# marionmari/pyGPs

Hardware: AMD Instinct MI355X
Metric: GP fits/sec (nlZ+grad, RBF, N=8192 d=16) (higher is better)
Workload: dtype f64; 1 GPU; GPR+RBF, N=8192 d=16 fp64 synthetic (SURVEY 8d recipe, seed 0), infExact nlZ + dnlZ (BASELINE configs[1]); x,y resident in HBM, hyp changes every step; outputs nlZ, dnlZ(4), alpha(N) to host per step; fits_per_rank=313, fit_streams_per_gpu=2, sched=1

## Files before the change

### pygps_amd/_lib.py

```python
import ctypes as C
import os
import threading

import numpy as np

_HERE = os.path.dirname(os.path.abspath(__file__))
LIB_PATH = os.environ.get("PYGPS_AMD_LIB") or os.path.join(_HERE, "libpygps_amd.so")

COV_RBF, COV_RBFARD, COV_MATERN, COV_RBFUNIT, COV_RQ, COV_PIECEPOLY = 0, 1, 2, 3, 4, 5
COV_RQARD, COV_GABOR, COV_PERIODIC, COV_NOISE, COV_CONST, COV_SM = 6, 7, 8, 9, 10, 11
COV_PRE = 12
COV_LINEAR, COV_POLY, COV_LINARD = 13, 14, 15
COV_COMPOSITE = 100
PROG_LEAF, PROG_SUM, PROG_PRODUCT, PROG_SCALE = 1, 2, 3, 4
PROG_MAX_ARD_DIM = 64
PROG_MAX = 8
MODE_TRAIN, MODE_CROSS, MODE_SELF_TEST = 0, 1, 2
LIK_ERF, LIK_GAUSS, LIK_LAPLACE = 0, 1, 2
ERR_LAPLACE_WNEG = -90
ERR_PROP_NONFINITE = -91
ERR_XU_UNSUPPORTED = -92
PROP_NONE, PROP_T, PROP_SPREAD = 0, 1, 2
PROP_MAX_LABELS = 256
PROP_SORT_LDS = 2048
# ... 78 lines not shown
    "pgp_profile_read": (C.c_int, [_vp, C.c_int, C.POINTER(_i64), _dp, _dp, _dp]),
    "pgp_profile_reset": (C.c_int, [_vp]),
    "pgp_set_option": (C.c_int, [_vp, C.c_char_p, C.c_int]),
    "pgp_comm_unique_id": (C.c_int, [C.c_char_p, C.c_char_p]),
    "pgp_comm_init_rccl": (C.c_int, [_vp, C.c_int, C.c_int, C.c_char_p, C.c_char_p, C.POINTER(_vp)]),
    "pgp_comm_init_host": (C.c_int, [_vp, C.c_int, C.c_int, _vp, _vp, _vp, C.POINTER(_vp)]),
    "pgp_comm_free": (None, [_vp]),
    "pgp_comm_world": (C.c_int, [_vp]),
    "pgp_comm_rank": (C.c_int, [_vp]),
    "pgp_comm_bcast_host": (C.c_int, [_vp, _dp, _i64, C.c_int]),
    "pgp_comm_allreduce_host": (C.c_int, [_vp, _dp, _i64, C.c_int]),
    "pgp_comm_allgather_host": (C.c_int, [_vp, _dp, _i64, _dp]),
    "pgp_sharded_exact_fit": (C.c_int, [_vp, _vp, C.c_int, _dp, C.c_int, C.c_int, C.c_int, C.c_double, _dp, _dp, C.c_int,
                                        C.c_int, _dp, _dp, _dp, _dp, _dp, C.POINTER(_vp)]),
    "pgp_sharded_predict": (C.c_int, [_vp, _vp, _vp, _dp, _i64, _dp, _dp, _dp]),
    "pgp_sfactor_free": (None, [_vp, _vp]),
    "pgp_sfactor_bytes": (_i64, [_vp]),
}

TEST_SIGNATURES = {
    "pgp_test_gemm": (C.c_int, [_vp, C.c_int, C.c_int, C.c_int, C.c_int, C.c_int, C.c_int, C.c_int, C.c_double,
                                C.c_double, _dp, _i64, _dp, _i64, _dp, _i64, C.c_int, C.c_int, C.c_int, C.c_int,
                                _dp]),
    "pgp_test_gemm_shrink": (C.c_int, [_vp, _dp, _i64, C.c_int, C.c_int, C.c_int, C.c_int, C.c_int, C.c_int, _dp, _i64,
                                       _i64]),
    "pgp_test_gemm_zskip": (C.c_int, [_vp] + [C.c_int] * 5 + [C.c_double, C.c_double, _dp, _i64, _dp, _i64, _dp, _dp, _i64,
                                      C.c_int, C.c_int, C.c_int]),
    "pgp_test_gemm_pair": (C.c_int, [_vp, C.c_double, C.c_double, _dp, _i64, _dp, _i64, _dp, _dp, _i64, C.c_int, C.c_int, C.c_int,
                                     C.c_int]),
    "pgp_test_gemm_skip_wait": (C.c_int, [_vp, C.c_int, _dp, _dp, _dp, C.c_int, C.c_int, C.c_int, C.c_int, C.c_int,
                                          C.POINTER(C.c_int)]),
    "pgp_test_probit_hazard": (C.c_int, [_vp, _dp, _dp, C.c_int]),
    "pgp_test_laplace_lik": (C.c_int, [_vp, C.c_int, C.c_double, _dp, _dp, C.c_int, _dp]),
    "pgp_test_laplace_ep_lik": (C.c_int, [_vp, _dp, _dp, _dp, _dp, C.c_int, _dp]),
    "pgp_test_valu_peak": (C.c_int, [_vp, C.c_int, C.c_int, _dp]),
    "pgp_test_mfma_peak": (C.c_int, [_vp, C.c_int, _dp]),
    "pgp_test_mfma_cycles": (C.c_int, [_vp, C.c_int, C.c_int, C.c_int, _dp]),
    "pgp_test_leaf_ticks": (C.c_int, [_vp, _dp]),
    "pgp_test_assemble": (C.c_int, [_vp, C.c_int, C.c_int, _i64, _i64, C.c_int, _dp]),
    "pgp_test_gemm_trace": (C.c_int, [_vp, C.c_int, C.c_int, C.c_int, C.c_int, C.c_int, C.POINTER(C.c_longlong), _i64, C.POINTER(_i64)]),
    "pgp_test_read_gemm_trace": (C.c_int, [_vp, C.POINTER(C.c_longlong), _i64, C.POINTER(_i64)]),
    "pgp_test_store_roof": (C.c_int, [_vp, _i64, C.c_int, C.c_int, _dp]),
    "pgp_test_cumask_gemm": (C.c_int, [_vp, C.c_int, C.c_int, C.c_int, C.c_int, C.c_int, _dp]),
    "pgp_test_wave_costs": (C.c_int, [_vp, _dp]),
    "pgp_test_stream_concurrency": (C.c_int, [_vp, C.c_int, _dp]),
    "pgp_test_slot_probe": (C.c_int, [_vp, C.c_int, C.c_int, C.c_int, C.c_int, C.c_int, C.c_int, _dp]),
# ... 204 lines not shown
```

### pygps_amd/csrc/capi.hip

```cpp
#include <algorithm>
#include <atomic>
#include <cmath>
#include <cstdio>
#include <cstdlib>
#include <cstring>
#include <map>
#include <string>
#include <mutex>
#include <vector>

#include "ctx.h"

static thread_local char g_err[512] = "";
void pgp_set_last_hip_error(hipError_t e, const char* what, const char* file, int line) {
    snprintf(g_err, sizeof(g_err), "HIP error %d (%s) in %s at %s:%d", (int)e, hipGetErrorString(e), what, file, line);
    (void)hipGetLastError();
}

static void ctx_register(pgp_ctx* c);
static void ctx_unregister(pgp_ctx* c);

void prof_collect(pgp_ctx* c) {
    if (c->recs.empty()) return;
    (void)hipStreamSynchronize(c->st);
// ... 132 lines not shown
    (void)hipStreamDestroy(c->st);
    if (c->st2) (void)hipStreamDestroy(c->st2);
    delete c;
}

int pgp_device_info(pgp_ctx* c, int* n_cu, int* sclk_mhz, double* hbm_gib, char* name, int name_len) {
    if (!c) return -1;
    if (n_cu) *n_cu = c->prop.multiProcessorCount;
    if (sclk_mhz) *sclk_mhz = c->prop.clockRate / 1000;
    if (hbm_gib) *hbm_gib = (double)c->prop.totalGlobalMem / (1024.0 * 1024.0 * 1024.0);
    if (name && name_len > 0) { strncpy(name, c->prop.name, name_len - 1); name[name_len - 1] = 0; }
    return PGP_OK;
}

int pgp_set_option(pgp_ctx* c, const char* name, int value) {
    if (!c || !name) return -1;
    if (!strcmp(name, "nb_outer")) { if (value < 0) return -3; c->nb_outer = value; return PGP_OK; }
    if (!strcmp(name, "joint_refine")) { c->joint_refine = value != 0; return PGP_OK; }
    if (!strcmp(name, "small_tile_below")) { c->small_tile_below = value; return PGP_OK; }
    if (!strcmp(name, "trtri_small_tile_below")) { c->trtri_small_tile_below = value; return PGP_OK; }
    if (!strcmp(name, "xcd_order")) { c->xcd_order = value; return PGP_OK; }
    if (!strcmp(name, "gemm_dbg")) { if (value & ~(64 | 256 | 512)) return -2; c->gemm_dbg = value; return PGP_OK; }
    if (!strcmp(name, "tile_ring")) { if (value < 0 || value > 1) return -2; c->tile_ring = value; return PGP_OK; }
    if (!strcmp(name, "lookahead")) { c->lookahead = value; return PGP_OK; }
    if (!strcmp(name, "leaf_first")) { c->leaf_first = value; return PGP_OK; }
    if (!strcmp(name, "leaf_pivot")) { if (value < 0 || value > 2) return -2; c->leaf_pivot = value; return PGP_OK; }
    if (!strcmp(name, "sched")) { if (value < -1 || value > 2) return -2; c->sched = value < 0 ? PGP_SCHED_DEFAULT : value; c->sched_explicit = value >= 0; return PGP_OK; }
    if (!strcmp(name, "concurrent_streams")) { c->concurrent_streams = value != 0; return PGP_OK; }
    if (!strcmp(name, "tud_tile")) { if (value != 64 && value != 128) return -2; c->tud_tile = value; return PGP_OK; }
    if (!strcmp(name, "tur_tile")) { if (value != 0 && value != 64 && value != 128 && value != 1264) return -2; c->tur_tile = value; return PGP_OK; }
    if (!strcmp(name, "s_pan")) { if (value < -1 || value > 2) return -2; c->s_pan = value; return PGP_OK; }
    if (!strcmp(name, "s_pan_direct")) { c->s_pan_direct = value != 0; return PGP_OK; }
    if (!strcmp(name, "s_pan_out")) { c->s_pan_out = value != 0; return PGP_OK; }
    if (!strcmp(name, "skip_zeros")) { c->skip_zeros = value != 0; return PGP_OK; }
    if (!strcmp(name, "tud_mark")) { c->tud_mark = value != 0; return PGP_OK; }
    if (!strcmp(name, "sched2_wide")) { c->sched2_wide = value != 0; return PGP_OK; }
    if (!strcmp(name, "gram_assembly")) { if (value < 0 || value > 2) return -2; c->gram_assembly = value; return PGP_OK; }
    if (!strcmp(name, "yield")) { c->yield = value; return PGP_OK; }
    if (!strcmp(name, "ep_fused")) { c->ep_fused = value; return PGP_OK; }
    if (!strcmp(name, "ep_tol_exp")) { if (value < 1 || value > 16) return -3; c->ep_tol_exp = value; return PGP_OK; }
    if (!strcmp(name, "ep_max_sweep")) { if (value < 2 || value > 1000) return -3; c->ep_max_sweep = value; return PGP_OK; }
    if (!strcmp(name, "laplace_tol_exp")) { if (value < 1 || value > 16) return -3; c->laplace_tol_exp = value; return PGP_OK; }
    if (!strcmp(name, "ep_r_direct")) { c->ep_r_direct = value; return PGP_OK; }
    if (!strcmp(name, "ep_alpha_direct")) { c->ep_alpha_direct = value; return PGP_OK; }
    if (!strcmp(name, "ep_sym")) { c->ep_sym = value; return PGP_OK; }
    if (!strcmp(name, "ep_wait_kernel")) { c->ep_wait_kernel = value; return PGP_OK; }
// ... 395 lines not shown
    for (long k = 0; k < c->d; ++k) bound += cs.scale[k] * cs.scale[k] * c->xdev2[k];
    return bound <= 64.0;
}

static int gemm_prepare(pgp_ctx* c, GemmArgs& g) {
    if (g.batch < 1) g.batch = 1;
    g.dbg |= c->gemm_dbg;
    bool xcd = false;
    if (c->xcd_order && !g.order && g.tile != 64 && g.tile != 1264 && g.batch == 1 && g.K <= c->xcd_max_k) {
        const long mt = g.M / 128, nt = g.N / 128;
        const long tiles = g.tri == 2 ? mt * (mt + 1) / 2 : (g.tri == 1 ? mt * nt - nt * (nt - 1) / 2 : mt * nt);
        xcd = tiles >= c->xcd_min_tiles;
    }
    if (g.tri == 1 && !g.order && !xcd) {
        const int T = g.tile == 64 ? 64 : 128;
        CHK(tri_tile_list(c, g.M / T, g.N / T, g.tri_off / T, &g.order, &g.norder));
    }
    if (xcd) CHK(tile_order(c, g.M / 128, g.N / 128, g.tri, g.tri ? g.tri_off / 128 : 0, &g.order, &g.norder));
    if (c->yield && c->yield_flags) {
        g.yield_flags = c->yield_flags;
        if (g.yield_role != 2) g.yield_role = gemm_f64_uses_dma(g) ? 1 : 0;
    } else g.yield_role = 0;
    g.ring = c->tile_ring && gemm_f64_uses_dma(g) ? 1 : 0;
    if (c->gemm_trace && gemm_f64_uses_dma128(g) && g.batch == 1) {
        const long mt = g.M / 128, nt = g.N / 128;
        const long nb = g.order ? g.norder : (g.tri == 2 ? mt * (mt + 1) / 2 : mt * nt);
        if (c->gemm_trace_pos + nb <= c->gemm_trace_cap) { g.trace = c->gemm_trace + 8 * c->gemm_trace_pos; c->gemm_trace_pos += nb; }
    }
    return PGP_OK;
}

int gemm_prof(pgp_ctx* c, int cls, GemmArgs g, hipStream_t st) {
    if (!st) st = c->st;
    CHK(gemm_prepare(c, g));
    ProfScope ps(c, cls, g.flops, 0.0, st, gemm_f64_uses_dma128(g) ? PC_KERNEL_DMA128 : -1);
    return gemm_f64_launch(g, st);
}

int gemm_prof_pair(pgp_ctx* c, int cls_a, GemmArgs a, int cls_b, GemmArgs b, hipStream_t st) {
    if (!st) st = c->st;
    CHK(gemm_prepare(c, a));
    CHK(gemm_prepare(c, b));
    if (c->pair_launch && gemm_f64_pair_ok(a, b)) {
        ProfScope ps(c, cls_a, a.flops + b.flops, 0.0, st, PC_KERNEL_DMA128);
        return gemm_f64_launch_pair(a, b, st);
    }
// ... 635 lines not shown
```

### pygps_amd/csrc/common.h

```cpp
#pragma once
#include <hip/hip_runtime.h>
#include <cstdint>
#include <cstdio>

#define PGP_OK 0
#define PGP_ERR_HIP (-100)
#define PGP_ERR_ARG (-1)

#define HIP_TRY(expr)                                                                       \
    do {                                                                                    \
        hipError_t e__ = (expr);                                                            \
        if (e__ != hipSuccess) {                                                            \
            pgp_set_last_hip_error(e__, #expr, __FILE__, __LINE__);                         \
            return PGP_ERR_HIP;                                                             \
        }                                                                                   \
    } while (0)

void pgp_set_last_hip_error(hipError_t e, const char* what, const char* file, int line);

enum GemmKMode {
    KM_FULL = 0,
    KM_GE_I = 1,
    KM_GE_J = 2,
    KM_LT_I = 3,
    KM_LT_J = 4,
};

struct GemmArgs {
    const double* A; long lda; int a_kc;
    const double* B; long ldb; int b_kc;
    double* C; long ldc;
    int M, N, K;
    double alpha, beta;
    int tri;
    int tri_off;
    int mask_diag;
    int kmode; int koff;
    int batch; long sA, sB, sC;
    int tile;
    const int* order;
    int norder;
    int order_z;
    int dbg;
    int ring;
    double flops;
    const double* A2; long lda2; int a_split;
    double* C2; long ldc2; int c_split;
    const double* Cin; long ldcin; const double* Cin2; long ldcin2;
    int rev_cols;
    int rev_rows;
    int fold_rows;
    int zero_from;
    int zf_upper;
    int batch_dm;
    int batch_dk;
    int batch_dldc; long batch_sC2;
    unsigned* yield_flags; int yield_role;
    int skip_lo, skip_hi;
    unsigned* wait_flag; unsigned wait_target; unsigned* wait_err;
    long long* trace;
};

__device__ __forceinline__ unsigned pgp_cu_key() {
    const unsigned hw = __builtin_amdgcn_s_getreg((4 << 0) | (0 << 6) | (31 << 11));
    const unsigned xcc = __builtin_amdgcn_s_getreg((20 << 0) | (0 << 6) | (3 << 11)) & 15u;
    return (xcc << 8) | ((hw >> 8) & 0xffu);
}
__device__ __forceinline__ void pgp_yield_mark(unsigned* flags, int delta) {
    if (flags && threadIdx.x == 0) {
        if (delta > 0) __hip_atomic_fetch_add(flags + pgp_cu_key(), 1u, __ATOMIC_RELAXED, __HIP_MEMORY_SCOPE_AGENT);
        else __hip_atomic_fetch_sub(flags + pgp_cu_key(), 1u, __ATOMIC_RELAXED, __HIP_MEMORY_SCOPE_AGENT);
    }
}

int gemm_f64_launch(const GemmArgs& g, hipStream_t st);
bool gemm_f64_pair_ok(const GemmArgs& a, const GemmArgs& b);
int gemm_f64_launch_pair(const GemmArgs& a, const GemmArgs& b, hipStream_t st);
bool gemm_f64_uses_dma(const GemmArgs& g);
bool gemm_f64_uses_dma128(const GemmArgs& g);

void func_max_dynamic_lds(const void* fn, size_t bytes);
```

### pygps_amd/csrc/ctx.h

```cpp
#pragma once
#include <algorithm>
#include <atomic>
#include <chrono>
#include <condition_variable>
#include <cstdio>
#include <cstdlib>
#include <map>
#include <mutex>
#include <vector>

#include "../../include/pygps_amd.h"
#include "kernels.h"
#include "sqdist_tile.h"

enum ProfClass { PC_ASSEMBLE = 0, PC_GEMM_TRAIL, PC_GEMM_INNER, PC_LEAF, PC_TRSM, PC_LEAFINV, PC_GEMM_TRTRI,
                 PC_GEMM_LAUUM, PC_HADAMARD, PC_SMALL, PC_GEMM_SOLVE, PC_DIAG, PC_KERNEL_DMA128, PC_COUNT };
static const char* const kProfNames[PC_COUNT] = {
    "cov_tile_kernel(assemble)", "gemm_f64(potrf trailing syrk)", "gemm_f64(potrf inner update)",
    "leaf_potrf_kernel", "trsm_rows_kernel", "leaf_inv_kernel", "gemm_f64(trtri)", "gemm_f64(lauum W^T W)",
    "hadamard_reduce_kernel", "small/O(N) kernels", "gemm_f64(panel solve X E_D)", "diag_in/out staging",
    "kernel gemm_f64_kernel<128,128,false,false,true,*> + gemm_f64_pair_kernel (LDS-DMA 128-tile)"};

struct ProfRec { int cls; hipEvent_t e0, e1; double flops, bytes; int shadow; };

// ... 101 lines not shown
    double *Dk = nullptr, *dpack = nullptr, *Xs = nullptr;
    int xcd_max_k = 512;
    int xcd_min_tiles = 256;
    int xcd_super = 8;
    int solve_outer = 8;
    int keep_inverse = 1;
    int predict_inverse = 1;
    int joint_refine = 1;
    int predict_batch = 65536;
    int s_tile = 0;
    int gram_fast = 2, gram_grid = 32768;
    int asm_grid = 4096, asm_nt = 0;
    size_t Xs_bytes = 0;
    hipEvent_t ev[PGP_NSTAGE + 2];
    double last_ms[PGP_NSTAGE];
    bool prof = false;
    std::vector<ProfRec> recs;
    std::vector<hipEvent_t> ev_pool;
    double pc_ms[PC_COUNT], pc_flops[PC_COUNT], pc_bytes[PC_COUNT];
    int64_t pc_launch[PC_COUNT];
    std::map<std::vector<int>, std::pair<int*, int>> orders;
    int gemm_dbg = 64 | 256 | 512;
    int tile_ring = 1;
    int xcd_order = 0;
    int nb_outer = 0;
    int trtri_small_tile_below = 2049;
    int small_tile_below = 200;
};

#define CHK(x)                      \
    do {                            \
        int rc__ = (x);             \
        if (rc__ != PGP_OK) return rc__; \
    } while (0)

int pgp_ctx_count_on_device(int device);
void pgp_drop_idle_pools(int device);

static inline bool pool_trace_on() { static const bool on = getenv("PGP_POOL_TRACE") != nullptr; return on; }
static inline hipError_t pool_hip_malloc(void** out, size_t bytes, const char* who) {
    if (!pool_trace_on()) return hipMalloc(out, bytes);
    const auto t0 = std::chrono::steady_clock::now();
    const hipError_t e = hipMalloc(out, bytes);
    fprintf(stderr, "[pool] hipMalloc %8.1f MiB  %8.3f ms  (%s)%s\n", bytes / 1048576.0,
            std::chrono::duration<double, std::milli>(std::chrono::steady_clock::now() - t0).count(), who, e == hipSuccess ? "" : " FAILED");
    return e;
// ... 282 lines not shown
```

### pygps_amd/csrc/gemm_f64.hip

```cpp
#include <algorithm>
#include <atomic>

#include "gemm_tile.h"

void func_max_dynamic_lds(const void* fn, size_t bytes) {
    constexpr int MAXF = 64, MAXD = 16;
    static std::atomic<const void*> fns[MAXF];
    static std::atomic<size_t> done[MAXF][MAXD];
    int dev = 0;
    if (hipGetDevice(&dev) != hipSuccess || dev < 0 || dev >= MAXD) { (void)hipFuncSetAttribute(fn, hipFuncAttributeMaxDynamicSharedMemorySize, (int)bytes); return; }
    int slot = -1;
    for (int i = 0; i < MAXF; ++i) {
        const void* cur = fns[i].load(std::memory_order_acquire);
        if (cur == fn) { slot = i; break; }
        if (cur == nullptr) {
            const void* expect = nullptr;
            if (fns[i].compare_exchange_strong(expect, fn, std::memory_order_acq_rel) || expect == fn) { slot = i; break; }
        }
    }
    if (slot < 0) { (void)hipFuncSetAttribute(fn, hipFuncAttributeMaxDynamicSharedMemorySize, (int)bytes); return; }
    if (done[slot][dev].load(std::memory_order_acquire) >= bytes) return;
    (void)hipFuncSetAttribute(fn, hipFuncAttributeMaxDynamicSharedMemorySize, (int)bytes);
    size_t prev = done[slot][dev].load(std::memory_order_relaxed);
    while (prev < bytes && !done[slot][dev].compare_exchange_weak(prev, bytes, std::memory_order_release)) {}
// ... 6 lines not shown

__device__ __forceinline__ bool decode_tile(const GemmArgs& g, int b, int T, int TNc, int& ti, int& tj) {
    if (g.order) {
        ti = g.order[2 * b];
        tj = g.order[2 * b + 1];
        return ti >= 0;
    }
    if (g.tri == 2) {
        int r = (int)((sqrt(8.0 * (double)b + 1.0) - 1.0) * 0.5);
        while ((long)(r + 1) * (r + 2) / 2 <= b) ++r;
        while ((long)r * (r + 1) / 2 > b) --r;
        ti = r;
        tj = b - r * (r + 1) / 2;
        return true;
    }
    const int mt = g.M / T;
    ti = b % mt;
    tj = b / mt;
    if (g.rev_cols) tj = g.N / TNc - 1 - tj;
    if (g.rev_rows) ti = mt - 1 - ti;
    return true;
}

template <int TM, int TN, bool AKC, bool BKC, bool DMA = false, bool YIELD = false, bool RING = false>
__global__ __launch_bounds__(256, 2) void gemm_f64_kernel(GemmArgs g) {
    extern __shared__ __attribute__((aligned(16))) double smem[];
    if (g.trace) {
        long long* tr0 = g.trace + 8L * (blockIdx.x + (long)gridDim.x * blockIdx.z);
        tr0[0] = (long long)wall_clock64();
        tr0[6] = (long long)__builtin_readcyclecounter();
    }
    int ti, tj;
    if (!decode_tile(g, (int)blockIdx.x, TM, TN, ti, tj)) return;
    long bz = blockIdx.z;
    if (g.order_z) { bz = ti >> 16; ti &= 0xffff; }
    if (g.wait_flag) {
        if (threadIdx.x == 0) {
            for (unsigned it = 0; (int)(__hip_atomic_load(g.wait_flag, __ATOMIC_ACQUIRE, __HIP_MEMORY_SCOPE_AGENT) - g.wait_target) < 0; ++it) {
                if (it > (1u << 22) || ((it & 1023u) == 1023u && __hip_atomic_load(g.wait_err, __ATOMIC_RELAXED, __HIP_MEMORY_SCOPE_AGENT))) {
                    __hip_atomic_store(g.wait_err, 1u, __ATOMIC_RELAXED, __HIP_MEMORY_SCOPE_AGENT);
                    break;
                }
                __builtin_amdgcn_s_sleep(8);
            }
        }
        __syncthreads();
    }
    if (!YIELD && g.yield_role == 2) {
        pgp_yield_mark(g.yield_flags, +1);
        gemm_tile_ns::gemm_tile<TM, TN, AKC, BKC, DMA, false, RING>(g, ti, tj, bz, smem, (int)(blockIdx.x + gridDim.x * blockIdx.z));
        __syncthreads();
        pgp_yield_mark(g.yield_flags, -1);
        return;
    }
    gemm_tile_ns::gemm_tile<TM, TN, AKC, BKC, DMA, YIELD, RING>(g, ti, tj, bz, smem, (int)(blockIdx.x + gridDim.x * blockIdx.z));
}

template <bool YIELD, bool RING = false>
__global__ __launch_bounds__(256, 2) void gemm_f64_pair_kernel(GemmArgs a, GemmArgs b, int na) {
    extern __shared__ __attribute__((aligned(16))) double smem[];
    auto run = [&](const GemmArgs& g, int bid) {
        if (g.trace) {
            long long* tr0 = g.trace + 8L * bid;
            tr0[0] = (long long)wall_clock64();
            tr0[6] = (long long)__builtin_readcyclecounter();
        }
        int ti, tj;
        if (!decode_tile(g, bid, 128, 128, ti, tj)) return;
        gemm_tile_ns::gemm_tile<128, 128, false, false, true, YIELD, RING>(g, ti, tj, 0, smem, bid);
    };
    if ((int)blockIdx.x < na) run(a, (int)blockIdx.x);
    else run(b, (int)blockIdx.x - na);
}

template <bool YIELD, bool RING = false>
__global__ __launch_bounds__(256, 2) void gemm_f64_fold_kernel(GemmArgs g) {
    extern __shared__ __attribute__((aligned(16))) double smem[];
    const int mt = g.M / 128, half = (mt + 1) / 2;
    const int r = (int)blockIdx.x % half, tj = (int)blockIdx.x / half;
    const int hi = mt - 1 - r;
    const long bz = blockIdx.z;
    gemm_tile_ns::gemm_tile<128, 128, false, false, true, YIELD, RING>(g, hi, tj, bz, smem, 0);
    if (hi != r) {
        __syncthreads();
        gemm_tile_ns::gemm_tile<128, 128, false, false, true, YIELD, RING>(g, r, tj, bz, smem, 0);
    }
}

constexpr size_t DMA_SPARE = 16;

template <int T, bool AKC, bool BKC, bool DMA = false, bool YIELD = false, bool RING = false>
int launch_t(const GemmArgs& g, hipStream_t st) {
    constexpr int SK = BK + 2;
    constexpr int ASZ = AKC ? T * SK : BK * (T + 16);
    constexpr int BSZ = BKC ? T * SK : BK * (T + 16);
    const size_t shm = 2 * (ASZ + BSZ) * sizeof(double) + (DMA ? DMA_SPARE : 0);
    const int mt = g.M / T, nt = g.N / T;
    unsigned nblk = (g.tri == 2) ? (unsigned)((long)mt * (mt + 1) / 2) : (unsigned)(mt * nt);
    if (g.order) nblk = (unsigned)g.norder;
    dim3 grid(nblk, 1, (g.batch > 0 && !g.order_z) ? g.batch : 1);
    func_max_dynamic_lds((const void*)gemm_f64_kernel<T, T, AKC, BKC, DMA, YIELD, RING>, shm);
    hipLaunchKernelGGL((gemm_f64_kernel<T, T, AKC, BKC, DMA, YIELD, RING>), grid, dim3(256), shm, st, g);
    return hipGetLastError() == hipSuccess ? PGP_OK : PGP_ERR_HIP;
}

static bool dma_ok(const GemmArgs& g);
static bool dma1264_ok(const GemmArgs& g) {
    return g.tile == 1264 && dma_ok(g) && !g.tri && !g.order && g.batch <= 1 && !g.order_z && (g.N % 64) == 0 && (g.M % 128) == 0 && g.kmode == KM_FULL;
}
template <bool YIELD, bool RING>
int launch_1264(const GemmArgs& g, hipStream_t st) {
    constexpr int SA_ = 128 + 16;
    const size_t shm = 2 * (BK * SA_ + (BK / 2) * SA_) * sizeof(double) + DMA_SPARE;
    dim3 grid((unsigned)((g.M / 128) * (g.N / 64)), 1, 1);
    func_max_dynamic_lds((const void*)gemm_f64_kernel<128, 64, false, false, true, YIELD, RING>, shm);
    hipLaunchKernelGGL((gemm_f64_kernel<128, 64, false, false, true, YIELD, RING>), grid, dim3(256), shm, st, g);
    return hipGetLastError() == hipSuccess ? PGP_OK : PGP_ERR_HIP;
}

static bool dma_ok(const GemmArgs& g) {
    return g.tile != 64 && (g.dbg & 64) && !g.a_kc && !g.b_kc && (g.K % 16) == 0 && (g.koff % 16) == 0 && (g.batch_dk % 16) == 0;
}

template <int T>
int launch_l(const GemmArgs& g, hipStream_t st) {
    if (!g.a_kc && !g.b_kc) return launch_t<T, false, false>(g, st);
    if (!g.a_kc && g.b_kc) return launch_t<T, false, true>(g, st);
    if (g.a_kc && !g.b_kc) return launch_t<T, true, false>(g, st);
    return launch_t<T, true, true>(g, st);
}

}

bool gemm_f64_uses_dma128(const GemmArgs& g) { return dma_ok(g) && !dma1264_ok(g); }
bool gemm_f64_uses_dma(const GemmArgs& g) { return dma_ok(g); }

static unsigned launch_blocks(const GemmArgs& g) {
    const int mt = g.M / 128, nt = g.N / 128;
    if (g.order) return (unsigned)g.norder;
    return (g.tri == 2) ? (unsigned)((long)mt * (mt + 1) / 2) : (unsigned)(mt * nt);
}
bool gemm_f64_pair_ok(const GemmArgs& a, const GemmArgs& b) {
    auto plain = [](const GemmArgs& g) {
        return g.M > 0 && g.N > 0 && g.tile != 64 && dma_ok(g) && g.batch <= 1 && !g.order_z && !g.wait_flag && g.yield_role != 2;
    };
    return plain(a) && plain(b) && (a.yield_role == 1 && a.yield_flags) == (b.yield_role == 1 && b.yield_flags) && !a.ring == !b.ring;
}
int gemm_f64_launch_pair(const GemmArgs& a, const GemmArgs& b, hipStream_t st) {
    if (!gemm_f64_pair_ok(a, b)) return -2;
    constexpr int SA_ = 128 + 16;
    const size_t shm = 2 * (2 * BK * SA_) * sizeof(double) + DMA_SPARE;
    const unsigned na = launch_blocks(a), nb = launch_blocks(b);
    const bool yield = a.yield_role == 1 && a.yield_flags;
    auto go = [&](auto kern) {
        func_max_dynamic_lds((const void*)kern, shm);
        hipLaunchKernelGGL(kern, dim3(na + nb), dim3(256), shm, st, a, b, (int)na);
    };
// ... 37 lines not shown
```

### pygps_amd/csrc/gemm_tile.h

```cpp
#pragma once
#include "common.h"

typedef double double4_t __attribute__((ext_vector_type(4)));
typedef double double2_t __attribute__((ext_vector_type(2)));

namespace gemm_tile_ns {

constexpr int BK = 16;

template <int LDS_OFF>
__device__ __forceinline__ void lds_dma_1k_s(unsigned voff, const double* sbase, unsigned lds_wave_base) {
    asm volatile("s_add_u32 m0, %2, %3\n\ts_nop 0\n\tglobal_load_lds_dwordx4 %0, %1"
                 :: "v"(voff), "s"(sbase), "s"(lds_wave_base), "n"(LDS_OFF) : "memory", "scc");
}
__device__ __forceinline__ const double* uniform_ptr(const double* p) {
    const unsigned long a = (unsigned long)p;
    const unsigned lo = __builtin_amdgcn_readfirstlane((unsigned)a), hi = __builtin_amdgcn_readfirstlane((unsigned)(a >> 32));
    return (const double*)(((unsigned long)hi << 32) | lo);
}
template <int V> struct IC { static constexpr int value = V; };

template <int N>
__device__ __forceinline__ void ring_wait() { asm volatile("s_waitcnt vmcnt(%0)" :: "n"(N) : "memory"); }
template <int N>
// ... 1 lines not shown
    asm volatile("s_waitcnt vmcnt(%0) lgkmcnt(0)" :: "n"(N) : "memory");
    __builtin_amdgcn_s_barrier();
    asm volatile("" ::: "memory");
}
__device__ __forceinline__ void ring_load_f64(double& d, const double* p) {
    asm volatile("global_load_dwordx2 %0, %1, off" : "=v"(d) : "v"(p) : "memory");
}
__device__ __forceinline__ void ring_landed(double& d) { asm volatile("" : "+v"(d)); }
__device__ __forceinline__ void ring_landed(unsigned& d) { asm volatile("" : "+v"(d)); }

__device__ __forceinline__ double swap_adjacent(double v) {
    const int lo = __builtin_amdgcn_update_dpp(0, __double2loint(v), 0xB1, 0xF, 0xF, false);
    const int hi = __builtin_amdgcn_update_dpp(0, __double2hiint(v), 0xB1, 0xF, 0xF, false);
    return __hiloint2double(hi, lo);
}

__device__ __noinline__ void gemm_yield_wait(const unsigned* yf) {
    for (int i = 0; i < 400; ++i) {
        __builtin_amdgcn_s_sleep(32);
        if (__hip_atomic_load(yf, __ATOMIC_RELAXED, __HIP_MEMORY_SCOPE_AGENT) == 0u) break;
    }
}

template <int TM, int TN, bool AKC, bool BKC, bool DMA = false, bool YIELD = false, bool RING = false>
__device__ __forceinline__ void gemm_tile(const GemmArgs& g, int ti, int tj, long bz, double* __restrict__ smem, int wg = 0) {
    static_assert(!RING || DMA, "the staging ring is an LDS-DMA loop");
    static_assert(!DMA || (!AKC && !BKC && TM == 128 && (TN == 128 || TN == 64)), "LDS-DMA staging: M-contiguous operands, 128 x 128 or 128 x 64 tiles");
    constexpr bool BH = DMA && TN == 64;
    constexpr int SA = TM + 16, SB = BH ? TM + 16 : TN + 16, SK = BK + 2;
    constexpr int ASZ = AKC ? TM * SK : BK * SA;
    constexpr int BSZ = BKC ? TN * SK : (BH ? (BK / 2) * SB : BK * SB);
    constexpr int STAGE = ASZ + BSZ;
    constexpr int FM = TM / 32, FN = TN / 32;
    constexpr int AV = TM * BK / 2 / 256;
    constexpr int BV = TN * BK / 2 / 256;

    const int i0 = ti * TM, j0 = tj * TN;
    if (g.batch_dm && i0 >= g.M - (int)bz * g.batch_dm) return;
    const int zero_from = g.zero_from > 0 ? g.zero_from - (int)bz * g.batch_dm : 0;
    if (i0 < g.skip_hi && j0 < g.skip_hi && i0 >= g.skip_lo && j0 >= g.skip_lo) return;
    bool diag = false;
    if (g.tri) {
        if (i0 + g.tri_off < j0) return;
        diag = g.mask_diag && (i0 + g.tri_off == j0);
    }
    int k0 = 0, k1 = g.K;
    const int koff = g.koff + (int)bz * g.batch_dk;
    if (g.kmode == KM_GE_I) k0 = i0 + koff;
    else if (g.kmode == KM_GE_J) k0 = j0 + koff;
// ... 141 lines not shown
                *(double2_t*)(sa + kr * SA + 2 * mv) = ra[p];
            }
        } else {
#pragma unroll
            for (int p = 0; p < AV; ++p) {
                const int kp = t & 7, m = (t >> 3) + p * 32;
                *(double2_t*)(sa + m * SK + 2 * kp) = ra[p];
            }
        }
        if (!BKC) {
            constexpr int VPR = TN / 2;
            constexpr int RPP = 256 / VPR;
#pragma unroll
            for (int p = 0; p < BV; ++p) {
                const int nv = t % VPR, kr = t / VPR + p * RPP;
                *(double2_t*)(sb + kr * SB + 2 * nv) = rb[p];
            }
        } else {
#pragma unroll
            for (int p = 0; p < BV; ++p) {
                const int kp = t & 7, n = (t >> 3) + p * 32;
                *(double2_t*)(sb + n * SK + 2 * kp) = rb[p];
            }
        }
    };

    double cr[8];
    const int ring_half = __builtin_amdgcn_readfirstlane(wave >> 1);
    auto ring_cact = [&](int fold_step) __attribute__((always_inline)) { return !BH || ring_half == (fold_step >> 3); };
    auto ring_cload = [&](int chunk) __attribute__((always_inline)) {
        const int in = chunk / (FM / 2), hf = chunk % (FM / 2);
#pragma unroll
        for (int q = 0; q < 2; ++q) {
            const double* cp = Cin + (long)(i0 + wm + (2 * hf + q) * 16 + l15) + (long)(j0 + wn + in * 16 + l4) * ldcin;
#pragma unroll
            for (int r = 0; r < 4; ++r) ring_load_f64(cr[4 * q + r], cp + (long)(4 * r) * ldcin);
        }
    };
    if (k0 < k1) {
        if constexpr (RING) {
            ring_issue(IC<0>{}, IC<0>{});
            ring_issue(IC<0>{}, IC<1>{});
            if (k0 + BK < k1) {
                ring_issue(IC<1>{}, IC<0>{});
                if (lazyc && ring_cact(1)) { ring_cload(0); ring_wait_barrier<2 * P + 8>(); }
                else ring_wait_barrier<2 * P>();
            } else ring_wait_barrier<P>();
        } else {
        if constexpr (DMA) {
            dma_stage(IC<0>{});
            asm volatile("s_waitcnt vmcnt(0)" ::: "memory");
        } else {
            gload(k0);
            sstore(0);
        }
        __syncthreads();
        }
        double fa[2][FM], fb[2][FN];
        auto ldfrag = [&](int b, int ks, int slot) {
            const double* sa = smem + b * STAGE;
            const double* sb = sa + ASZ;
            const int k = ks * 4 + l4;
#pragma unroll
            for (int im = 0; im < FM; ++im) {
                const int m = wm + im * 16 + l15;
                fa[slot][im] = AKC ? sa[m * SK + k] : sa[k * SA + m];
            }
#pragma unroll
            for (int in = 0; in < FN; ++in) {
                const int n = wn + in * 16 + l15;
                if constexpr (BH) fb[slot][in] = sb[(l4 + 4 * (ks >> 1)) * SB + (ks & 1) * 64 + n];
                else fb[slot][in] = BKC ? sb[n * SK + k] : sb[k * SB + n];
            }
        };
        auto mfmas = [&](int slot) {
#pragma unroll
            for (int in = 0; in < FN; ++in)
#pragma unroll
                for (int im = 0; im < FM; ++im)
// ... 130 lines not shown
                    if (!(st & 1)) {
                        if (act) {
#pragma unroll
                        for (int q = 0; q < 2; ++q) {
                            const double* cp = Cin + (long)(i0 + wm + (2 * hf + q) * 16 + l15) + (long)(j0 + wn + in * 16 + l4) * ldcin;
#pragma unroll
                            for (int r = 0; r < 4; ++r) creg[q][r] = cp[(long)(4 * r) * ldcin];
                        }
                        }
                    } else if (act) {
#pragma unroll
                        for (int q = 0; q < 2; ++q)
#pragma unroll
                            for (int r = 0; r < 4; ++r) acc[2 * hf + q][in][r] = fma(ab, creg[q][r], acc[2 * hf + q][in][r]);
                    }
                    if (st & 1) kstep(kt, IC<1>{}, IC<0>{});
                    else if ((st & 3) == 0) kstep(kt, IC<0>{}, IC<1>{});
                    else kstep(kt, IC<0>{}, IC<0>{});
                    kt += BK;
                }
                if (g.trace) smem[2 * STAGE] = __longlong_as_double((long long)wall_clock64());
            }
        }
        while (kt < k1) {
            kstep(kt, IC<0>{}, IC<1>{});
            kt += BK;
            if (kt >= k1) break;
            kstep(kt, IC<1>{}, IC<0>{});
            kt += BK;
            if constexpr (YIELD) {
                if (kt >= k1) break;
                kstep(kt, IC<0>{}, IC<0>{});
                kt += BK;
                if (kt >= k1) break;
                kstep(kt, IC<1>{}, IC<0>{});
                kt += BK;
            }
        }
        }
    }

    long long* const trc = g.trace ? g.trace + 8L * wg : nullptr;
    if (trc) {
        trc[2] = (long long)wall_clock64();
        if constexpr (DMA) trc[1] = lazyc ? __double_as_longlong(smem[2 * STAGE]) : 0ll;
    }
// ... 42 lines not shown
```

### pygps_amd/csrc/testhooks.h

```cpp
#pragma once
#include <stdint.h>

#include "../../include/pygps_amd.h"
#ifdef __cplusplus
extern "C" {
#endif
int pgp_test_gemm(pgp_ctx* ctx, int tile, int a_kc, int b_kc, int tri, int mask_diag, int kmode, int koff,
                  double alpha, double beta, const double* A, int64_t lda, const double* B, int64_t ldb,
                  double* C, int64_t ldc, int M, int N, int K, int iters, double* ms_out);
int pgp_test_gemm_shrink(pgp_ctx* ctx, const double* Y, int64_t ldy, int M, int K, int w, int nb, int dm, int zero_from,
                         double* C, int64_t ldc, int64_t sC);
int pgp_test_gemm_zskip(pgp_ctx* ctx, int tile, int tri, int mask_diag, int zero_from, int zf_upper, double alpha, double beta,
                        const double* A, int64_t lda, const double* B, int64_t ldb, const double* Cin, double* C, int64_t ldc,
                        int M, int N, int K);
int pgp_test_gemm_pair(pgp_ctx* ctx, double alpha, double beta, const double* A, int64_t lda, const double* B, int64_t ldb, double* Ca,
                       double* Cb, int64_t ldc, int M, int N, int Ka, int Kb);
int pgp_test_gemm_skip_wait(pgp_ctx* ctx, int tile, const double* A, const double* B, double* C, int n, int K, int skip_lo,
                            int skip_hi, int wait_ms, int* timed_out);
int pgp_test_probit_hazard(pgp_ctx* ctx, const double* z, double* out, int n);
int pgp_test_laplace_lik(pgp_ctx* ctx, int lik, double log_sn, const double* y, const double* f, int n, double* out);
int pgp_test_laplace_ep_lik(pgp_ctx* ctx, const double* y, const double* mu, const double* s2, const double* sn, int n, double* out);
int pgp_test_valu_peak(pgp_ctx* ctx, int iters, int waves_per_simd, double* out2);
int pgp_test_mfma_peak(pgp_ctx* ctx, int iters, double* tflops_out);
int pgp_test_mfma_cycles(pgp_ctx* ctx, int iters, int nacc, int waves_per_simd, double* out3);
int pgp_test_leaf_ticks(pgp_ctx* ctx, double* ticks_out );
int pgp_test_wave_costs(pgp_ctx* ctx, double* out16);
int pgp_test_slot_probe(pgp_ctx* ctx, int nwg, int lds_kb, int hold_us, int reserve, int probe_lds_kb, int delay_us, double* out4);
int pgp_test_cumask_gemm(pgp_ctx* ctx, int M, int K, int reserve_per_xcd, int stride, int iters, double* out2);
int pgp_test_assemble(pgp_ctx* ctx, int kind, int mode, int64_t n, int64_t d, int iters, double* ms_out);
int pgp_test_gemm_trace(pgp_ctx* ctx, int M, int K, int tri, int warm, int conc, long long* out, int64_t out_words, int64_t* nblk_out);
int pgp_test_read_gemm_trace(pgp_ctx* ctx, long long* out, int64_t words, int64_t* nwg);
int pgp_test_store_roof(pgp_ctx* ctx, int64_t n, int grid, int iters, double* out3);
// ... 17 lines not shown
```

### pygps_amd/csrc/testhooks.hip

```cpp
#include <time.h>
#include <cstdlib>
#include <cmath>
#include <vector>

#include "ctx.h"
#include <chrono>
#include <thread>

#include "testhooks.h"
#include "erf_lik.h"
#include "laplace_lik.h"

typedef double double4_t __attribute__((ext_vector_type(4)));

namespace {
__global__ __launch_bounds__(256) void mfma_peak_kernel(double* out, int iters, double a0, double b0) {
    double4_t acc[8];
#pragma unroll
    for (int i = 0; i < 8; ++i) acc[i] = double4_t{0.0, 0.0, 0.0, 0.0};
    double a = a0 + threadIdx.x * 1e-9, b = b0;
    for (int it = 0; it < iters; ++it) {
#pragma unroll
        for (int i = 0; i < 8; ++i) acc[i] = __builtin_amdgcn_mfma_f64_16x16x4f64(a, b, acc[i], 0, 0, 0);
    }
// ... 345 lines not shown
    (void)hipEventDestroy(e0); (void)hipEventDestroy(e1);
    (void)hipFree(tab); (void)hipFree(out);
    return hipGetLastError() == hipSuccess ? PGP_OK : PGP_ERR_HIP;
}

int pgp_test_gemm(pgp_ctx* ctx, int tile, int a_kc, int b_kc, int tri, int mask_diag, int kmode, int koff,
                  double alpha, double beta, const double* A, int64_t lda, const double* B, int64_t ldb, double* C,
                  int64_t ldc, int M, int N, int K, int iters, double* ms_out) {
    if (!ctx) return -1;
    pgp_ctx* c = ctx;
    const bool poll = getenv("PGP_TEST_GEMM_YIELD") != nullptr;
    if (poll && !c->yield_flags) return -2;
    HIP_TRY(hipSetDevice(c->device));
    const size_t an = (size_t)lda * (a_kc ? M : K), bn = (size_t)ldb * (b_kc ? N : K), cn = (size_t)ldc * N;
    double *Ad, *Bd, *Cd;
    HIP_TRY(hipMalloc((void**)&Ad, an * 8)); HIP_TRY(hipMalloc((void**)&Bd, bn * 8)); HIP_TRY(hipMalloc((void**)&Cd, cn * 8));
    HIP_TRY(hipMemcpy(Ad, A, an * 8, hipMemcpyHostToDevice));
    HIP_TRY(hipMemcpy(Bd, B, bn * 8, hipMemcpyHostToDevice));
    HIP_TRY(hipMemcpy(Cd, C, cn * 8, hipMemcpyHostToDevice));
    GemmArgs g{};
    g.A = Ad; g.lda = lda; g.a_kc = a_kc; g.B = Bd; g.ldb = ldb; g.b_kc = b_kc; g.C = Cd; g.ldc = ldc;
    g.M = M; g.N = N; g.K = K; g.alpha = alpha; g.beta = beta; g.tri = tri; g.tri_off = 0; g.mask_diag = mask_diag;
    g.kmode = kmode; g.koff = koff; g.batch = 1; g.tile = tile; g.dbg = c->gemm_dbg; g.ring = c->tile_ring != 0;
    if (getenv("PGP_TEST_GEMM_FOLD")) g.fold_rows = 1;
    if (poll && gemm_f64_uses_dma(g)) { g.yield_flags = c->yield_flags; g.yield_role = 1; }
    hipStream_t ts = c->st;
    int rc = gemm_f64_launch(g, ts);
    HIP_TRY(hipStreamSynchronize(ts));
    if (rc == PGP_OK) HIP_TRY(hipMemcpy(C, Cd, cn * 8, hipMemcpyDeviceToHost));
    if (rc == PGP_OK && iters > 0 && ms_out) {
        hipEvent_t e0, e1;
        HIP_TRY(hipEventCreate(&e0)); HIP_TRY(hipEventCreate(&e1));
        {
            HIP_TRY(hipEventRecord(e0, ts));
            rc = gemm_f64_launch(g, ts);
            HIP_TRY(hipEventRecord(e1, ts));
            HIP_TRY(hipStreamSynchronize(ts));
            float m1 = 0.f;
            HIP_TRY(hipEventElapsedTime(&m1, e0, e1));
            const int nwarm = (int)std::min(4000.0, std::max(1.0, 80.0 / std::max(1e-3, (double)m1)));
            for (int i = 0; i < nwarm && rc == PGP_OK; ++i) rc = gemm_f64_launch(g, ts);
        }
        HIP_TRY(hipEventRecord(e0, ts));
        for (int i = 0; i < iters; ++i) rc = gemm_f64_launch(g, ts);
        HIP_TRY(hipEventRecord(e1, ts));
        HIP_TRY(hipStreamSynchronize(ts));
        float ms = 0.f;
        HIP_TRY(hipEventElapsedTime(&ms, e0, e1));
        *ms_out = ms / iters;
        (void)hipEventDestroy(e0); (void)hipEventDestroy(e1);
    }
    (void)hipFree(Ad); (void)hipFree(Bd); (void)hipFree(Cd);
    return rc;
}

int pgp_test_gemm_trace(pgp_ctx* c, int M, int K, int tri, int warm, int conc, long long* out, int64_t out_words, int64_t* nblk_out) {
    if (!c || !out || !nblk_out || M % 128 || K % 16) return -1;
    HIP_TRY(hipSetDevice(c->device));
    const long mt = M / 128;
    const long nblk = tri ? mt * (mt + 1) / 2 : mt * mt;
    if (out_words < 8 * nblk) return -2;
    double *A, *Cd, *C2; long long* tr;
    HIP_TRY(hipMalloc((void**)&A, (size_t)M * K * 8)); HIP_TRY(hipMalloc((void**)&Cd, (size_t)M * M * 8));
    HIP_TRY(hipMalloc((void**)&C2, (size_t)M * M * 8)); HIP_TRY(hipMalloc((void**)&tr, (size_t)nblk * 64));
    HIP_TRY(hipMemset(tr, 0, (size_t)nblk * 64));
    std::vector<double> h((size_t)M * K);
    unsigned long long s = 88172645463325252ULL;
    for (auto& v : h) { s ^= s << 13; s ^= s >> 7; s ^= s << 17; v = ((double)(s >> 11) / 9007199254740992.0 - 0.5) * 0.01; }
    HIP_TRY(hipMemcpy(A, h.data(), h.size() * 8, hipMemcpyHostToDevice));
    HIP_TRY(hipMemset(Cd, 0, (size_t)M * M * 8)); HIP_TRY(hipMemset(C2, 0, (size_t)M * M * 8));
    GemmArgs g{};
    g.A = A; g.lda = M; g.B = A; g.ldb = M; g.C = Cd; g.ldc = M; g.M = M; g.N = M; g.K = K; g.alpha = -1.0; g.beta = 1.0;
    g.tri = tri ? 2 : 0; g.mask_diag = tri ? 1 : 0; g.batch = 1; g.tile = 128; g.dbg = c->gemm_dbg; g.ring = c->tile_ring != 0;
    int rc = PGP_OK;
    for (int i = 0; i < warm && rc == PGP_OK; ++i) rc = gemm_f64_launch(g, c->st);
// ... 396 lines not shown
```

Before: 112.2 fits/s.

## Prefetch global tiles two stages ahead in the register-staged 64x64 GEMM

Adds an AHEAD variant of the 64x64 register-staged f64 GEMM tile. It keeps two sets of staging registers so global loads for the tile after next are issued while the current tile's MFMAs run, which hides more global-memory latency. The variant is enabled by default for tile=64 with a non-transposed A and a K-contiguous B, and its launch bounds go from 2 to 4 waves per unit. The extra staging registers combined with the tighter launch bound could cause spills. The change also adds a test hook for timing and tracing the solve-style GEMM.

```diff
diff --git a/pygps_amd/_lib.py b/pygps_amd/_lib.py
--- a/pygps_amd/_lib.py
+++ b/pygps_amd/_lib.py
@@ -124,6 +124,8 @@
     "pgp_test_gemm": (C.c_int, [_vp, C.c_int, C.c_int, C.c_int, C.c_int, C.c_int, C.c_int, C.c_int, C.c_double,
                                 C.c_double, _dp, _i64, _dp, _i64, _dp, _i64, C.c_int, C.c_int, C.c_int, C.c_int,
                                 _dp]),
+    "pgp_test_gemm_solve": (C.c_int, [_vp, C.c_int, C.c_int, C.c_int, C.c_int, _dp, _i64, _dp, _i64, _dp, _i64, _dp, _i64, C.c_int,
+                                      C.c_int, C.c_int, C.c_int, _dp, C.POINTER(C.c_longlong), _i64]),
     "pgp_test_gemm_shrink": (C.c_int, [_vp, _dp, _i64, C.c_int, C.c_int, C.c_int, C.c_int, C.c_int, C.c_int, _dp, _i64,
                                        _i64]),
     "pgp_test_gemm_zskip": (C.c_int, [_vp] + [C.c_int] * 5 + [C.c_double, C.c_double, _dp, _i64, _dp, _i64, _dp, _dp, _i64,
diff --git a/pygps_amd/csrc/capi.hip b/pygps_amd/csrc/capi.hip
--- a/pygps_amd/csrc/capi.hip
+++ b/pygps_amd/csrc/capi.hip
@@ -178,6 +178,7 @@
     if (!strcmp(name, "xcd_order")) { c->xcd_order = value; return PGP_OK; }
     if (!strcmp(name, "gemm_dbg")) { if (value & ~(64 | 256 | 512)) return -2; c->gemm_dbg = value; return PGP_OK; }
     if (!strcmp(name, "tile_ring")) { if (value < 0 || value > 1) return -2; c->tile_ring = value; return PGP_OK; }
+    if (!strcmp(name, "tile_ahead")) { if (value < 0 || value > 1) return -2; c->tile_ahead = value; return PGP_OK; }
     if (!strcmp(name, "lookahead")) { c->lookahead = value; return PGP_OK; }
     if (!strcmp(name, "leaf_first")) { c->leaf_first = value; return PGP_OK; }
     if (!strcmp(name, "leaf_pivot")) { if (value < 0 || value > 2) return -2; c->leaf_pivot = value; return PGP_OK; }
@@ -619,6 +620,7 @@
         if (g.yield_role != 2) g.yield_role = gemm_f64_uses_dma(g) ? 1 : 0;
     } else g.yield_role = 0;
     g.ring = c->tile_ring && gemm_f64_uses_dma(g) ? 1 : 0;
+    g.ahead = c->tile_ahead ? 1 : 0;
     if (c->gemm_trace && gemm_f64_uses_dma128(g) && g.batch == 1) {
         const long mt = g.M / 128, nt = g.N / 128;
         const long nb = g.order ? g.norder : (g.tri == 2 ? mt * (mt + 1) / 2 : mt * nt);
diff --git a/pygps_amd/csrc/common.h b/pygps_amd/csrc/common.h
--- a/pygps_amd/csrc/common.h
+++ b/pygps_amd/csrc/common.h
@@ -43,6 +43,7 @@
     int order_z;
     int dbg;
     int ring;
+    int ahead;
     double flops;
     const double* A2; long lda2; int a_split;
     double* C2; long ldc2; int c_split;
@@ -78,5 +79,6 @@
 int gemm_f64_launch_pair(const GemmArgs& a, const GemmArgs& b, hipStream_t st);
 bool gemm_f64_uses_dma(const GemmArgs& g);
 bool gemm_f64_uses_dma128(const GemmArgs& g);
+bool gemm_f64_uses_ahead(const GemmArgs& g);
 
 void func_max_dynamic_lds(const void* fn, size_t bytes);
diff --git a/pygps_amd/csrc/ctx.h b/pygps_amd/csrc/ctx.h
--- a/pygps_amd/csrc/ctx.h
+++ b/pygps_amd/csrc/ctx.h
@@ -147,6 +147,7 @@
     std::map<std::vector<int>, std::pair<int*, int>> orders;
     int gemm_dbg = 64 | 256 | 512;
     int tile_ring = 1;
+    int tile_ahead = 1;
     int xcd_order = 0;
     int nb_outer = 0;
     int trtri_small_tile_below = 2049;
diff --git a/pygps_amd/csrc/gemm_f64.hip b/pygps_amd/csrc/gemm_f64.hip
--- a/pygps_amd/csrc/gemm_f64.hip
+++ b/pygps_amd/csrc/gemm_f64.hip
@@ -52,8 +52,8 @@
     return true;
 }
 
-template <int TM, int TN, bool AKC, bool BKC, bool DMA = false, bool YIELD = false, bool RING = false>
-__global__ __launch_bounds__(256, 2) void gemm_f64_kernel(GemmArgs g) {
+template <int TM, int TN, bool AKC, bool BKC, bool DMA = false, bool YIELD = false, bool RING = false, bool AHEAD = false>
+__global__ __launch_bounds__(256, AHEAD ? 4 : 2) void gemm_f64_kernel(GemmArgs g) {
     extern __shared__ __attribute__((aligned(16))) double smem[];
     if (g.trace) {
         long long* tr0 = g.trace + 8L * (blockIdx.x + (long)gridDim.x * blockIdx.z);
@@ -78,12 +78,12 @@
     }
     if (!YIELD && g.yield_role == 2) {
         pgp_yield_mark(g.yield_flags, +1);
-        gemm_tile_ns::gemm_tile<TM, TN, AKC, BKC, DMA, false, RING>(g, ti, tj, bz, smem, (int)(blockIdx.x + gridDim.x * blockIdx.z));
+        gemm_tile_ns::gemm_tile<TM, TN, AKC, BKC, DMA, false, RING, AHEAD>(g, ti, tj, bz, smem, (int)(blockIdx.x + gridDim.x * blockIdx.z));
         __syncthreads();
         pgp_yield_mark(g.yield_flags, -1);
         return;
     }
-    gemm_tile_ns::gemm_tile<TM, TN, AKC, BKC, DMA, YIELD, RING>(g, ti, tj, bz, smem, (int)(blockIdx.x + gridDim.x * blockIdx.z));
+    gemm_tile_ns::gemm_tile<TM, TN, AKC, BKC, DMA, YIELD, RING, AHEAD>(g, ti, tj, bz, smem, (int)(blockIdx.x + gridDim.x * blockIdx.z));
 }
 
 template <bool YIELD, bool RING = false>
@@ -119,7 +119,7 @@
 
 constexpr size_t DMA_SPARE = 16;
 
-template <int T, bool AKC, bool BKC, bool DMA = false, bool YIELD = false, bool RING = false>
+template <int T, bool AKC, bool BKC, bool DMA = false, bool YIELD = false, bool RING = false, bool AHEAD = false>
 int launch_t(const GemmArgs& g, hipStream_t st) {
     constexpr int SK = BK + 2;
     constexpr int ASZ = AKC ? T * SK : BK * (T + 16);
@@ -129,8 +129,8 @@
     unsigned nblk = (g.tri == 2) ? (unsigned)((long)mt * (mt + 1) / 2) : (unsigned)(mt * nt);
     if (g.order) nblk = (unsigned)g.norder;
     dim3 grid(nblk, 1, (g.batch > 0 && !g.order_z) ? g.batch : 1);
-    func_max_dynamic_lds((const void*)gemm_f64_kernel<T, T, AKC, BKC, DMA, YIELD, RING>, shm);
-    hipLaunchKernelGGL((gemm_f64_kernel<T, T, AKC, BKC, DMA, YIELD, RING>), grid, dim3(256), shm, st, g);
+    func_max_dynamic_lds((const void*)gemm_f64_kernel<T, T, AKC, BKC, DMA, YIELD, RING, AHEAD>, shm);
+    hipLaunchKernelGGL((gemm_f64_kernel<T, T, AKC, BKC, DMA, YIELD, RING, AHEAD>), grid, dim3(256), shm, st, g);
     return hipGetLastError() == hipSuccess ? PGP_OK : PGP_ERR_HIP;
 }
 
@@ -154,6 +154,7 @@
 
 template <int T>
 int launch_l(const GemmArgs& g, hipStream_t st) {
+    if constexpr (T == 64) { if (gemm_f64_uses_ahead(g)) return launch_t<64, false, true, false, false, false, true>(g, st); }
     if (!g.a_kc && !g.b_kc) return launch_t<T, false, false>(g, st);
     if (!g.a_kc && g.b_kc) return launch_t<T, false, true>(g, st);
     if (g.a_kc && !g.b_kc) return launch_t<T, true, false>(g, st);
@@ -163,6 +164,7 @@
 }
 
 bool gemm_f64_uses_dma128(const GemmArgs& g) { return dma_ok(g) && !dma1264_ok(g); }
+bool gemm_f64_uses_ahead(const GemmArgs& g) { return g.ahead && g.tile == 64 && !g.a_kc && g.b_kc; }
 bool gemm_f64_uses_dma(const GemmArgs& g) { return dma_ok(g); }
 
 static unsigned launch_blocks(const GemmArgs& g) {
diff --git a/pygps_amd/csrc/gemm_tile.h b/pygps_amd/csrc/gemm_tile.h
--- a/pygps_amd/csrc/gemm_tile.h
+++ b/pygps_amd/csrc/gemm_tile.h
@@ -47,9 +47,10 @@
     }
 }
 
-template <int TM, int TN, bool AKC, bool BKC, bool DMA = false, bool YIELD = false, bool RING = false>
+template <int TM, int TN, bool AKC, bool BKC, bool DMA = false, bool YIELD = false, bool RING = false, bool AHEAD = false>
 __device__ __forceinline__ void gemm_tile(const GemmArgs& g, int ti, int tj, long bz, double* __restrict__ smem, int wg = 0) {
     static_assert(!RING || DMA, "the staging ring is an LDS-DMA loop");
+    static_assert(!AHEAD || (!DMA && !YIELD && TM == 64 && TN == 64), "two stages ahead: the register-staged 64 x 64 tile");
     static_assert(!DMA || (!AKC && !BKC && TM == 128 && (TN == 128 || TN == 64)), "LDS-DMA staging: M-contiguous operands, 128 x 128 or 128 x 64 tiles");
     constexpr bool BH = DMA && TN == 64;
     constexpr int SA = TM + 16, SB = BH ? TM + 16 : TN + 16, SK = BK + 2;
@@ -237,6 +238,28 @@
                 const int kp = t & 7, n = (t >> 3) + p * 32;
                 *(double2_t*)(sb + n * SK + 2 * kp) = rb[p];
             }
+        }
+    };
+    double2_t ra2[AHEAD ? AV : 1], rb2[AHEAD ? BV : 1];
+    auto gload_to = [&](double2_t (&a)[AV], double2_t (&b)[BV], bool adv) __attribute__((always_inline)) {
+        const long sa_ = adv ? astep : 0, sb_ = adv ? bstep : 0;
+#pragma unroll
+        for (int p = 0; p < AV; ++p) { pa[p] += sa_; a[p] = *(const double2_t*)pa[p]; }
+#pragma unroll
+        for (int p = 0; p < BV; ++p) { pb[p] += sb_; b[p] = *(const double2_t*)pb[p]; }
+    };
+    auto sstore_from = [&](int buf, const double2_t (&a)[AV], const double2_t (&b)[BV]) __attribute__((always_inline)) {
+        double* sa = smem + buf * STAGE;
+        double* sb = sa + ASZ;
+#pragma unroll
+        for (int p = 0; p < AV; ++p) {
+            if (!AKC) { constexpr int VPR = TM / 2, RPP = 256 / VPR; *(double2_t*)(sa + (t / VPR + p * RPP) * SA + 2 * (t % VPR)) = a[p]; }
+            else *(double2_t*)(sa + ((t >> 3) + p * 32) * SK + 2 * (t & 7)) = a[p];
+        }
+#pragma unroll
+        for (int p = 0; p < BV; ++p) {
+            if (!BKC) { constexpr int VPR = TN / 2, RPP = 256 / VPR; *(double2_t*)(sb + (t / VPR + p * RPP) * SB + 2 * (t % VPR)) = b[p]; }
+            else *(double2_t*)(sb + ((t >> 3) + p * 32) * SK + 2 * (t & 7)) = b[p];
         }
     };
 
@@ -265,11 +288,18 @@
         if constexpr (DMA) {
             dma_stage(IC<0>{});
             asm volatile("s_waitcnt vmcnt(0)" ::: "memory");
+        } else if constexpr (AHEAD) {
+            gload_to(ra, rb, false);
+            if (k0 + BK < k1) { gload_to(ra2, rb2, true); sstore_from(0, ra, rb); }
+            else sstore_from(0, ra, rb);
         } else {
             gload(k0);
             sstore(0);
         }
         __syncthreads();
+        if constexpr (!DMA && TM == 64 && TN == 64) {
+            if (g.trace) g.trace[8L * wg + 1] = (long long)wall_clock64();
+        }
         }
         double fa[2][FM], fb[2][FN];
         auto ldfrag = [&](int b, int ks, int slot) {
@@ -446,6 +476,31 @@
                 if (g.trace) smem[2 * STAGE] = __longlong_as_double((long long)wall_clock64());
             }
         }
+        if constexpr (AHEAD) {
+            auto astage = [&](auto bufc, auto ldc_, double2_t (&na)[AV], double2_t (&nb)[BV], double2_t (&fra)[AV], double2_t (&frb)[BV])
+                              __attribute__((always_inline)) {
+                constexpr int buf = decltype(bufc)::value, LD = decltype(ldc_)::value;
+                const bool more = kt + BK < k1;
+                if constexpr (LD != 0) gload_to(fra, frb, LD == 1 || kt + 2 * BK < k1);
+#pragma unroll
+                for (int ks = 0; ks + 1 < NS; ++ks) {
+                    ldfrag(buf, ks + 1, (ks + 1) & 1);
+                    mfmas(ks & 1);
+                }
+                if (LD != 0 || more) sstore_from(buf ^ 1, na, nb);
+                __syncthreads();
+                if (LD != 0 || more) ldfrag(buf ^ 1, 0, NS & 1);
+                __builtin_amdgcn_sched_barrier(0);
+                mfmas((NS - 1) & 1);
+                kt += BK;
+            };
+            while (kt + 2 * BK < k1) {
+                astage(IC<0>{}, IC<1>{}, ra2, rb2, ra, rb);
+                astage(IC<1>{}, IC<2>{}, ra, rb, ra2, rb2);
+            }
+            astage(IC<0>{}, IC<0>{}, ra2, rb2, ra, rb);
+            if (kt < k1) astage(IC<1>{}, IC<0>{}, ra, rb, ra2, rb2);
+        } else
         while (kt < k1) {
             kstep(kt, IC<0>{}, IC<1>{});
             kt += BK;
diff --git a/pygps_amd/csrc/testhooks.h b/pygps_amd/csrc/testhooks.h
--- a/pygps_amd/csrc/testhooks.h
+++ b/pygps_amd/csrc/testhooks.h
@@ -8,6 +8,9 @@
 int pgp_test_gemm(pgp_ctx* ctx, int tile, int a_kc, int b_kc, int tri, int mask_diag, int kmode, int koff,
                   double alpha, double beta, const double* A, int64_t lda, const double* B, int64_t ldb,
                   double* C, int64_t ldc, int M, int N, int K, int iters, double* ms_out);
+int pgp_test_gemm_solve(pgp_ctx* ctx, int koff, int c_split, int rev_cols, int ahead, const double* A, int64_t lda, const double* B,
+                        int64_t ldb, double* C, int64_t ldc, double* C2, int64_t ldc2, int M, int N, int K, int iters, double* ms_out,
+                        long long* trace_out, int64_t trace_words);
 int pgp_test_gemm_shrink(pgp_ctx* ctx, const double* Y, int64_t ldy, int M, int K, int w, int nb, int dm, int zero_from,
                          double* C, int64_t ldc, int64_t sC);
 int pgp_test_gemm_zskip(pgp_ctx* ctx, int tile, int tri, int mask_diag, int zero_from, int zf_upper, double alpha, double beta,
diff --git a/pygps_amd/csrc/testhooks.hip b/pygps_amd/csrc/testhooks.hip
--- a/pygps_amd/csrc/testhooks.hip
+++ b/pygps_amd/csrc/testhooks.hip
@@ -391,6 +391,7 @@
     g.A = Ad; g.lda = lda; g.a_kc = a_kc; g.B = Bd; g.ldb = ldb; g.b_kc = b_kc; g.C = Cd; g.ldc = ldc;
     g.M = M; g.N = N; g.K = K; g.alpha = alpha; g.beta = beta; g.tri = tri; g.tri_off = 0; g.mask_diag = mask_diag;
     g.kmode = kmode; g.koff = koff; g.batch = 1; g.tile = tile; g.dbg = c->gemm_dbg; g.ring = c->tile_ring != 0;
+    g.ahead = c->tile_ahead != 0;
     if (getenv("PGP_TEST_GEMM_FOLD")) g.fold_rows = 1;
     if (poll && gemm_f64_uses_dma(g)) { g.yield_flags = c->yield_flags; g.yield_role = 1; }
     hipStream_t ts = c->st;
@@ -420,6 +421,65 @@
         (void)hipEventDestroy(e0); (void)hipEventDestroy(e1);
     }
     (void)hipFree(Ad); (void)hipFree(Bd); (void)hipFree(Cd);
+    return rc;
+}
+
+int pgp_test_gemm_solve(pgp_ctx* c, int koff, int c_split, int rev_cols, int ahead, const double* A, int64_t lda, const double* B,
+                        int64_t ldb, double* C, int64_t ldc, double* C2, int64_t ldc2, int M, int N, int K, int iters, double* ms_out,
+                        long long* trace_out, int64_t trace_words) {
+    if (!c || !A || !B || !C || M <= 0 || N <= 0 || K <= 0 || (M % 64) || (N % 64) || (K % 16)) return -1;
+    if (c_split < 0 || c_split >= M || (c_split % 64) || (c_split > 0 && !C2) || lda < M || ldb < K) return -1;
+    const int m1 = c_split > 0 ? c_split : M, m2 = c_split > 0 ? M - c_split : 0;
+    if (ldc < m1 || (m2 > 0 && ldc2 < m2)) return -1;
+    const long nblk = (long)(M / 64) * (N / 64);
+    if (trace_out && trace_words < 8 * nblk) return -2;
+    HIP_TRY(hipSetDevice(c->device));
+    const size_t an = (size_t)lda * K, bn = (size_t)ldb * N, cn = (size_t)ldc * N, c2n = m2 > 0 ? (size_t)ldc2 * N : 0;
+    double *Ad = nullptr, *Bd = nullptr, *Cd = nullptr, *C2d = nullptr; long long* tr = nullptr;
+    auto release = [&]() { (void)hipFree(Ad); (void)hipFree(Bd); (void)hipFree(Cd); (void)hipFree(C2d); (void)hipFree(tr); };
+    auto run = [&]() -> int {
+        HIP_TRY(hipMalloc((void**)&Ad, an * 8)); HIP_TRY(hipMalloc((void**)&Bd, bn * 8)); HIP_TRY(hipMalloc((void**)&Cd, cn * 8));
+        if (m2 > 0) HIP_TRY(hipMalloc((void**)&C2d, c2n * 8));
+        HIP_TRY(hipMemcpy(Ad, A, an * 8, hipMemcpyHostToDevice));
+        HIP_TRY(hipMemcpy(Bd, B, bn * 8, hipMemcpyHostToDevice));
+        HIP_TRY(hipMemcpy(Cd, C, cn * 8, hipMemcpyHostToDevice));
+        if (m2 > 0) HIP_TRY(hipMemcpy(C2d, C2, c2n * 8, hipMemcpyHostToDevice));
+        GemmArgs g{};
+        g.A = Ad; g.lda = lda; g.a_kc = 0; g.B = Bd; g.ldb = ldb; g.b_kc = 1; g.C = Cd; g.ldc = ldc;
+        if (m2 > 0) { g.C2 = C2d; g.ldc2 = ldc2; g.c_split = c_split; }
+        g.M = M; g.N = N; g.K = K; g.alpha = 1.0; g.beta = 0.0; g.kmode = KM_LT_J; g.koff = koff; g.batch = 1; g.tile = 64;
+        g.rev_cols = rev_cols ? 1 : 0; g.dbg = c->gemm_dbg; g.ahead = ahead ? 1 : 0;
+        hipStream_t ts = c->st;
+        int rc = gemm_f64_launch(g, ts);
+        HIP_TRY(hipStreamSynchronize(ts));
+        if (rc != PGP_OK) return rc;
+        HIP_TRY(hipMemcpy(C, Cd, cn * 8, hipMemcpyDeviceToHost));
+        if (m2 > 0) HIP_TRY(hipMemcpy(C2, C2d, c2n * 8, hipMemcpyDeviceToHost));
+        if (iters > 0 && ms_out) {
+            hipEvent_t e0, e1;
+            HIP_TRY(hipEventCreate(&e0)); HIP_TRY(hipEventCreate(&e1));
+            for (int i = 0; i < 1500 && rc == PGP_OK; ++i) rc = gemm_f64_launch(g, ts);
+            HIP_TRY(hipEventRecord(e0, ts));
+            for (int i = 0; i < iters && rc == PGP_OK; ++i) rc = gemm_f64_launch(g, ts);
+            HIP_TRY(hipEventRecord(e1, ts));
+            HIP_TRY(hipStreamSynchronize(ts));
+            float ms = 0.f;
+            HIP_TRY(hipEventElapsedTime(&ms, e0, e1));
+            *ms_out = ms / iters;
+            (void)hipEventDestroy(e0); (void)hipEventDestroy(e1);
+        }
+        if (trace_out && rc == PGP_OK) {
+            HIP_TRY(hipMalloc((void**)&tr, (size_t)nblk * 64));
+            HIP_TRY(hipMemsetAsync(tr, 0, (size_t)nblk * 64, ts));
+            g.trace = tr;
+            rc = gemm_f64_launch(g, ts);
+            HIP_TRY(hipStreamSynchronize(ts));
+            HIP_TRY(hipMemcpy(trace_out, tr, (size_t)nblk * 64, hipMemcpyDeviceToHost));
+        }
+        return rc;
+    };
+    const int rc = run();
+    release();
     return rc;
 }
 
```

Result: no change. 111.8 fits/s (-0.3%).
